# SchusterLab/quantum-optimal-control

Measured on AMD Instinct MI355X. Metric: GRAPE iterations/sec (fwd+bwd+Adam) at n=32 k=4 steps=500, higher is better.
Workload: dtype f64; 1 GPU; C2 3-transmon-size unitary gate: n=32 k=4 steps=500 m=8 Taylor(T,s)=(5,3), 64 independent control seeds per GPU (aggregate over seeds), reg_coeffs={}; seeds_per_gpu=64, total_seeds=64, chunks=16, stream_groups=1, ranks_seen=1, fidelities_gathered=64, devices_distinct=1, transport=single process, transport_fallback=False

## Files before the change

### quantum-optimal-control_amd/csrc/qoc_engine.hip

```cpp
#include "../../include/qoc.h"

#include <hip/hip_runtime.h>

#include <cmath>
#include <cstdarg>
#include <cstdio>
#include <cstdlib>
#include <cstring>
#include <memory>
#include <string>
#include <type_traits>
#include <vector>

#include "qoc_common.h"
#include "qoc_kernels_finish.h"
#include "qoc_kernels_generic.h"
#include "qoc_kernels_mfma.h"
#include "qoc_kernels_st.h"
#include "qoc_kernels_gemm.h"
#include "qoc_gemm_ts.h"
#include "qoc_small.h"
#include "qoc_ensemble.h"
#include "qoc_transfer.h"
#include "qoc_control_map.h"
// ... 1741 lines not shown
}

int qoc_get_member_weights(qoc_handle e, double* pi) {
    CHECK_H(e);
    if (!e->ens_E) return fail(QOC_ERR_STATE, "qoc_get_member_weights: not an ensemble engine (qoc_create_ensemble, qoc_create_shaped)");
    if (!pi) return fail(QOC_ERR_INVALID, "qoc_get_member_weights: null output");
    const size_t E = (size_t)e->ens_E, cnt = (size_t)e->g.B * E;
    if (!risk_on(e)) {
        for (size_t i = 0; i < cnt; ++i) pi[i] = e->ens_wt[i % E];
        return QOC_OK;
    }
    HIP_TRY(hipStreamSynchronize(e->stream));
    HIP_TRY(hipMemcpy(pi, e->risk_pi, cnt * sizeof(double), hipMemcpyDeviceToHost));
    return QOC_OK;
}

int qoc_get_trajectory_gradient(qoc_handle e, double* dLdu) {
    CHECK_H(e);
    if (!e->ens_E) return fail(QOC_ERR_STATE, "qoc_get_trajectory_gradient: not an ensemble engine (qoc_create_ensemble)");
    if (!dLdu) return fail(QOC_ERR_INVALID, "qoc_get_trajectory_gradient: null output");
    if (!e->evaluated) return fail(QOC_ERR_STATE, "qoc_get_trajectory_gradient: nothing evaluated yet");
    HIP_TRY(hipStreamSynchronize(e->stream));
    HIP_TRY(hipMemcpy(dLdu, e->d.dLdu, (size_t)e->d.B * e->d.k * e->d.steps * sizeof(double), hipMemcpyDeviceToHost));
    return QOC_OK;
}

int qoc_get_member_final_unitary(qoc_handle e, double* Uf) {
    CHECK_H(e);
    if (!e->ens_E) return fail(QOC_ERR_STATE, "qoc_get_member_final_unitary: not an ensemble engine (qoc_create_ensemble)");
    if (e->lb.on) return fail(QOC_ERR_STATE, "qoc_get_member_final_unitary: an open engine has no final unitary (qoc_get_member_final_density)");
    if (!Uf) return fail(QOC_ERR_INVALID, "qoc_get_member_final_unitary: null output");
    if (e->d.state_transfer) return fail(QOC_ERR_STATE, "qoc_get_member_final_unitary: state-transfer mode has no final unitary");
    if (!e->evaluated) return fail(QOC_ERR_STATE, "qoc_get_member_final_unitary: nothing evaluated yet");
    TRY(refresh_final(e));
    HIP_TRY(hipStreamSynchronize(e->stream));
    HIP_TRY(hipMemcpy(Uf, e->d.Xfinal, (size_t)e->d.B * e->d.n * e->d.n * sizeof(cplx), hipMemcpyDeviceToHost));
    return QOC_OK;
}

int qoc_profile_enable(qoc_handle e, int32_t on) {
    CHECK_H(e);
    TRY(prof_collect(e));
    e->profiling = on != 0;
    e->prof_ms = 0.0;
    e->prof_launches = 0;
    return QOC_OK;
}

int qoc_profile_read(qoc_handle e, const char** kernel_name, int64_t* launches, double* total_ms) {
    CHECK_H(e);
    TRY(prof_collect(e));
    if (kernel_name)
        *kernel_name = e->path == QOC_PATH_SPARSE ? "k_sp_forward" : e->path == QOC_PATH_LINDBLAD ? "k_lb_forward" : e->path == QOC_PATH_SMALL ? "k_small_iter (whole iterations)"
                       : e->path == QOC_PATH_GEMM ? (e->gm.route == QOC_GEMM_DIRECT ? "k_gemm_taylor_chain (backward chain + sources + gradient products)"
                           : e->gm.N <= 64 ? "k_gemm_expm_fused (+ product tree)" : "k_zgemm_wg + k_zgemm32 (batched matexp sequence)")
                       : e->path == QOC_PATH_MFMA ? e->mp.expm_name
                       : e->path == QOC_PATH_ST_FUSED ? "k_st_fwd_fused" : (e->d.state_transfer ? "k_st_fwd_generic" : "k_expm_generic");
    if (launches) *launches = e->prof_launches;
    if (total_ms) *total_ms = e->prof_ms;
    return QOC_OK;
}

int qoc_time_iterations(qoc_handle e, const qoc_adam_params* p, int32_t iters, double* elapsed_ms) {
    CHECK_H(e);
    HIP_TRY(hipStreamSynchronize(e->stream));
    HIP_TRY(hipEventRecord(e->t0, e->stream));
    TRY(qoc_iterate(e, p, iters));
    HIP_TRY(hipEventRecord(e->t1, e->stream));
    HIP_TRY(hipEventSynchronize(e->t1));
    float ms = 0.f;
    HIP_TRY(hipEventElapsedTime(&ms, e->t0, e->t1));
    if (elapsed_ms) *elapsed_ms = ms;
    return QOC_OK;
}

int qoc_path_in_use(qoc_handle e) { return e ? e->path : QOC_ERR_INVALID; }
int qoc_chunks_in_use(qoc_handle e) { return e ? e->chunks : QOC_ERR_INVALID; }

int qoc_plan_describe(qoc_handle e, char* buf, int32_t len) {
    if (!e || !buf || len < 1) return fail(QOC_ERR_INVALID, "qoc_plan_describe: null handle or buffer");
    char tmp[768];
    if (e->path == QOC_PATH_MFMA) {
        int w = snprintf(tmp, sizeof tmp, "path=mfma nt=%d expm=%d chunks=%d sweeps=%s", e->mf.NT, e->mp.expm_variant, e->mf.C, e->mp.sweeps);
        if (e->mp.expm_variant == 8) w += snprintf(tmp + w, sizeof tmp - w, " expm_hermitian=%d", e->mp.expm_hermitian);
        snprintf(tmp + w, sizeof tmp - w, " mem_policy=%d", e->mp.mem_policy);
    } else if (e->path == QOC_PATH_GEMM) {
        const QocGemm& g = e->gm;
        const bool direct = g.route == QOC_GEMM_DIRECT;
        int w = snprintf(tmp, sizeof tmp, "path=gemm route=%s chunks=%d slices_per_chunk=%d chains=%s",
                         direct ? "direct" : (e->d.state_transfer ? "propagator" : "unitary"), g.NC, g.S, qoc_gemm_chain_routes(g) ? "persistent" : "launches");
        if (g.ts_G > 0) w += snprintf(tmp + w, sizeof tmp - w, " time_shards=%d time_rank=%d", g.ts_G, g.ts_rank);
        if (direct) snprintf(tmp + w, sizeof tmp - w, " taylor_chain=%s",
                             g.sq_chain ? "squared" : g.dpp_packed ? "packed"
                             : g.dpp_chain ? (g.dpp_cw == 10 ? "columns40" : g.dpp_cw == 12 ? "columns48" : g.dpp_cw == 14 ? "columns56" : "full")
                             : "butterfly");
    } else if (e->path == QOC_PATH_LINDBLAD) {
        snprintf(tmp, sizeof tmp, "path=lindblad collapse=%d pairs=%d lds=%zu", e->lb.c, e->lb.R, e->lb.lds_bytes);
    } else if (e->path == QOC_PATH_SPARSE) {
        const QocSparse& sp = e->sp;
        int w = snprintf(tmp, sizeof tmp, "path=sparse nnz=%lld ell=", sp.stored);
        for (size_t j = 0; j < e->sp_widths.size() && w < 320; ++j) w += snprintf(tmp + w, sizeof tmp - w, j ? ",%d" : "%d", e->sp_widths[j]);
        w += snprintf(tmp + w, sizeof tmp - w, " vector_home=%s lds=%zu threads=%d grad_grid=%d", sp.home == 1 ? "lds" : "global", sp.lds_bytes, sp.threads, sp.grad_grid);
        if (e->sp_fleet_entry) snprintf(tmp + w, sizeof tmp - w, " rows=%s merged_width=%d", sp.merged ? "merged" : "per_operator", sp.Wm);
    } else if (e->path == QOC_PATH_SMALL) {
        snprintf(tmp, sizeof tmp, "path=small n_pad=%d rows=%d slices_per_row=%d workgroups=%d state_sources=%d lds_kb=%d", e->sm.N, e->sm.R, e->sm.L, e->sm.G,
            e->sm.src ? 1 : 0, (int)((e->sm.lds_bytes + 1023) / 1024));
    } else {
        snprintf(tmp, sizeof tmp, "path=%s", e->path == QOC_PATH_ST_FUSED ? "st_fused" : "generic");
    }
    auto add = [&tmp](const char* fmt, auto... a) { const size_t w = strlen(tmp); snprintf(tmp + w, sizeof tmp - w, fmt, a...); };
    const int ks = sets(e).k * sets(e).steps;
    const TailKind tail = tail_kind(e);
    if (tail == TAIL_IN_LAUNCH) add(" tail=%s", "in_launch");
    else if (tail == TAIL_SPLIT) add(" tail=split%d", e->fin_S);
    else if (tail == TAIL_SPLIT_PARTIALS) add(" tail=split%d_partials", e->fin_S);
    else if (tail == TAIL_LATENCY_FUSED) add(" tail=latency_fused_%s", ks <= QF_E * (int)e->mp.grad_lat.block.x ? "regs" : "memory");
    else {
        const int threads = ks >= 2048 ? 1024 : QOC_BLOCK, qfe = tail == TAIL_FINISH8 ? 8 : QF_E;
        add(" tail=finish%d_%s", threads, tail == TAIL_FINISH8 ? "regs8" : (ks <= qfe * threads ? "regs" : "memory"));
    }
    if (e->ens_E) add(" members=%d perturbations=%d", e->ens_E, e->en.q);
    if (e->fleet_F) add(" devices=%d", e->fleet_F);
    if (e->shaped) add(" samples=%d band=%d", e->sh.P, e->sh.band);
    if (e->mapped) add(" terms=%d degree=%d", e->cm.r, e->cm.D);
    add(" gradient=%s", e->xg.on ? "exact" : "first_order");
    if (e->xg.on) add(" exact_variant=%s exact_lds=%zu exact_grid=%d", e->xg.lds ? "lds" : "global", e->xg.lds_bytes, e->xg.grid);
    if (e->lb.on && e->lb.nc > 0) add(" running_costs=%d", e->lb.nc);
    if (e->en.tr) add(" traces=1");
    snprintf(buf, (size_t)len, "%s", tmp);
    return QOC_OK;
}

}

#include "qoc_comm.h"
```

### quantum-optimal-control_amd/csrc/qoc_mfma_backward.hip

```cpp
#include "qoc_kernels_mfma.h"
#include "qoc_plan_limits.h"
#include "qoc_mfma_backward.h"
#include "qoc_mfma_downup.h"

template <int NT>
static const char* qoc_resolve_backward(QocMfmaPlan& p, const QocMfma& mf, const QocDev& d, bool split_grad, int mem_policy) {
    const unsigned items = d.B * mf.C, g4 = (items + 3) / 4, slices = d.B * d.steps;
    const bool src = d.n_forb > 0 || d.has_speed, fast = mf.variant != 1;
    const QocOneOf<2, 4> mq{mf.mq <= 2 ? 2 : 4};
    const QocOneOf<5, 4> kc{d.k == 5 ? 5 : 4};
    const QocOneOf<8, 7, 6, 5> qa{qoc_active_strips(d.n)};
    if (src && mf.C > 1) {
        const unsigned wpg = mf.lat_sources ? 1 : 4;
        if (NT == 2 && fast) qoc_pick([&](auto MQ, auto QA) { p.offsets.set(k_mfma_bwd_offsets2<MQ, false, QA>, (items + wpg - 1) / wpg, 64 * wpg); }, mq, qa);
        else p.offsets.set(k_mfma_bwd_offsets<NT>, g4, 256);
    }
    if constexpr (NT == 2) if (fast && d.k <= 5) {
        if (mf.lat_sources) {
            qoc_pick([&](auto MQ, auto KC) {
                p.sweep_groups.set(k_mfma_backward3<MQ, true, KC, 2>, d.B * mf.NG, 128, mf.bwd_lds3);
                p.sweep.set(k_mfma_backward3<MQ, true, KC, 1>, items, 128, mf.bwd_lds3);
            }, mq, kc);
            return p.sweep_groups.reserve() && p.sweep.reserve() ? nullptr : "MFMA path: cannot reserve LDS for the two-level backward kernel";
        }
// ... 44 lines not shown
        C = NT == 2 ? QOC_PLAN_CHUNK_ITEMS / d.Bplan : (QOC_PLAN_CHUNK_ITEMS + d.Bplan - 1) / d.Bplan;
        if (C > (NT == 2 ? QOC_PLAN_CHUNKS_MAX_NT2 : QOC_PLAN_CHUNKS_MAX)) C = NT == 2 ? QOC_PLAN_CHUNKS_MAX_NT2 : QOC_PLAN_CHUNKS_MAX;
    }
    mf.latency = mf.variant == 5;
    if (mf.latency && chunks_req <= 0) C = (d.steps + 7) / 8;
    if (C > d.steps) C = d.steps;
    if (C > (mf.latency ? 16 * QOC_MAXC : QOC_MAXC)) C = mf.latency ? 16 * QOC_MAXC : QOC_MAXC;
    if (C < 1) C = 1;
    int L = (d.steps + C - 1) / C;
    C = (d.steps + L - 1) / L;
    mf.C = C; mf.L = L;
    mf.G = 0; mf.NG = 0;
    mf.lat_sources = mf.latency && (d.n_forb > 0 || d.has_speed);
    if (mf.latency) {
        int G = 8;
        while (G * G < C) ++G;
        mf.G = G; mf.NG = (C + G - 1) / G;
    }
    mf.mq = (d.m + 3) / 4;
    {
        double f = 1.0;
        for (int j = 0; j < 24; ++j) { if (j > 0) f *= (double)j; mf.invfact[j] = 1.0 / f; }
    }
    std::vector<cplx> hd((size_t)(d.k + 1) * FR), ht((size_t)(d.k + 1) * FR), u0(FR);
    for (int kk = 0; kk <= d.k; ++kk) {
        qoc_to_fragD(Hs_host + (size_t)kk * d.n * d.n, d.n, false, hd.data() + (size_t)kk * FR, NT);
        qoc_to_fragD(Hs_host + (size_t)kk * d.n * d.n, d.n, true, ht.data() + (size_t)kk * FR, NT);
    }
    std::vector<cplx> u0h((size_t)d.n * d.n);
    if (hipMemcpy(u0h.data(), d.U0, u0h.size() * sizeof(cplx), hipMemcpyDeviceToHost) != hipSuccess) { msg = "U0 readback failed"; return -2; }
    qoc_to_fragD(u0h.data(), d.n, false, u0.data(), NT);
    auto up = [&](cplx** dst, const std::vector<cplx>& src) -> bool {
        void* p = nullptr;
        if (hipMalloc(&p, src.size() * sizeof(cplx)) != hipSuccess) return false;
        allocs.push_back(p);
        if (hipMemcpy(p, src.data(), src.size() * sizeof(cplx), hipMemcpyHostToDevice) != hipSuccess) return false;
        *dst = (cplx*)p;
        return true;
    };
    if (!up(&mf.HfD, hd) || !up(&mf.HfT, ht) || !up(&mf.U0fD, u0)) { msg = "MFMA path: constant upload failed"; return -3; }
    {
        const int T = d.T < 1 ? 1 : (d.T > 22 ? 22 : d.T);
        mf.psigma = std::pow(mf.invfact[T], 1.0 / (double)T);
        for (int j = 0; j < 24; ++j) mf.pcoef[j] = mf.invfact[j] * std::pow(mf.psigma, -(double)j);
        mf.pcoef[T] = 1.0;
        const double sc = mf.psigma / (double)(1 << d.s);
        std::vector<cplx> hs(hd);
        for (auto& v : hs) { v.x *= sc; v.y *= sc; }
        if (!up(&mf.HsD, hs)) { msg = "MFMA path: constant upload failed"; return -3; }
    }
    std::vector<std::pair<cplx**, size_t>> wanted;
    auto al = [&](cplx** dst, size_t count) -> bool { wanted.emplace_back(dst, (count * sizeof(cplx) + 4095) & ~(size_t)4095); return true; };
    mf.skew_c = 5 * 16;
    mf.skew_b = 3 * 16;
    const size_t nk = (size_t)d.B * ((size_t)d.steps * FR + (size_t)C * mf.skew_c + mf.skew_b), np = (size_t)d.B * C * FR;
    mf.store_T = !((NT == 2 || NT == 3) && mf.variant != 1) || mf.latency;
    const bool split_grad = (NT > 2 || (NT == 2 && d.k >= 6)) && mf.variant != 1;
    if (split_grad && !al(&mf.LamD, (size_t)d.B * d.steps * 16 * NT * 16)) { msg = "MFMA path: out of device memory"; return -3; }
    { const int kg = NT >= 4 ? 2 : 4; mf.grad_lds = (size_t)(d.k < kg ? d.k : kg) * FR * sizeof(cplx); }
    mf.grad_rt = NT >= 2 && split_grad && d.k <= 8 && !qoc_exp_is("QOC_GRAD_RT", 0);
    if (mf.grad_rt) {
        mf.grad_lds = (size_t)((d.k + 3) & ~3) * NT * 256 * sizeof(cplx);
        if (!al((cplx**)&mf.gpart, ((size_t)NT * d.B * d.k * d.steps + 1) / 2)) { msg = "MFMA path: out of device memory"; return -3; }
    }
    if (mf.updown && !al(&mf.LamL, (size_t)d.B * d.steps * NT * (mf.mq <= 2 ? 2 : 4) * 64)) { msg = "MFMA path: out of device memory"; return -3; }
    if (mf.lat_sources && !al(&mf.Goff, (size_t)d.B * mf.NG * 4 * NT * 64)) { msg = "MFMA path: out of device memory"; return -3; }
    const bool bnd = (NT == 2 || NT == 3) && mf.variant != 1 && !mf.latency;
    const bool bnd_adj = bnd && NT == 2 && d.k <= 5 && !(d.n_forb > 0 || d.has_speed);
    mf.updown = mf.updown && bnd_adj;
    const size_t nbnd = (size_t)d.B * C * NT * (mf.mq <= 2 ? 2 : 4) * 64;
    if ((bnd && !al(&mf.BndF, nbnd)) || (bnd_adj && !al(&mf.BndA, nbnd))) { msg = "MFMA path: out of device memory"; return -3; }
    const bool dressed = d.n_forb > 0 && d.forbid_dressed;
    mf.lat_src_fast = mf.lat_sources && !(dressed && d.n_forb > 4);
    mf.lat_dressed = mf.lat_src_fast && dressed;
    if (mf.lat_src_fast) {
        const size_t vec = (size_t)NT * (mf.mq <= 2 ? 2 : 4) * 64;
        if (!al(&mf.AoffL, (size_t)d.B * C * vec) || !al(&mf.GoffL, (size_t)d.B * mf.NG * vec) || !al(&mf.LamS, (size_t)d.B * d.steps * vec) ||
            !al((cplx**)&mf.loss_part, (size_t)d.B * (d.steps + 1))) { msg = "MFMA path: out of device memory"; return -3; }
    }
    if (mf.latency && (!al(&mf.GfD, (size_t)d.B * mf.NG * FR) || !al(&mf.GfT, (size_t)d.B * mf.NG * FR) || !al(&mf.TfD, (size_t)d.B * FR) ||
                       !al(&mf.PsiL, (size_t)d.B * d.steps * NT * (mf.mq <= 2 ? 2 : 4) * 64) ||
                       !al(&mf.LamL, (size_t)d.B * d.steps * NT * (mf.mq <= 2 ? 2 : 4) * 64))) { msg = "MFMA path: out of device memory"; return -3; }
    if (!al(&mf.KfD, nk) || (mf.store_T && !al(&mf.KfT, nk)) || !al(&mf.PfD, np) || !al(&mf.PfT, np) || !al(&mf.Aoff, (size_t)d.B * C * 4 * NT * 64)) { msg = "MFMA path: out of device memory"; return -3; }
    {
        size_t total = 0;
        for (auto& w : wanted) total += w.second;
        char* arena = nullptr;
        if (hipMalloc((void**)&arena, qoc_arena_bytes(total)) != hipSuccess) { msg = "MFMA path: out of device memory"; return -3; }
        allocs.push_back(arena);
        size_t off = 0;
        for (auto& w : wanted) { *w.first = (cplx*)(arena + off); off += w.second; }
        const size_t xl = (size_t)d.B * d.steps * NT * (mf.mq <= 2 ? 2 : 4) * 64 * sizeof(cplx);
        if (mf.PsiL && (hipMemset(mf.PsiL, 0, xl) != hipSuccess || hipMemset(mf.LamL, 0, xl) != hipSuccess)) { msg = "MFMA path: clearing PsiL / LamL failed"; return -2; }
        if (NT == 2 && d.n <= 28 && (hipMemset(mf.KfD, 0, nk * sizeof(cplx)) != hipSuccess || (mf.KfT && hipMemset(mf.KfT, 0, nk * sizeof(cplx)) != hipSuccess))) {
            msg = "MFMA path: clearing the propagator buffers failed"; return -2;
        }
    }
    const size_t pads = (size_t)4 * 16 * (16 * NT + 1) * sizeof(cplx);
    const size_t hbytes = (size_t)d.k * FR * sizeof(cplx);
    mf.h_in_lds = (hbytes + pads) <= 160 * 1024;
    mf.bwd_lds = pads + (mf.h_in_lds ? hbytes : 0);
    {
        const int kc = d.k == 5 ? 5 : 4;
        mf.bwd_lds3 = (size_t)kc * FR * sizeof(cplx) + (size_t)8 * 2 * 16 * B2_LDP * sizeof(cplx) + 4 * 2 * 2 * 4 * kc * sizeof(double);
    }
    if (mf.latency) {
        void* p = nullptr;
        if (hipMalloc(&p, (size_t)d.B * sizeof(unsigned)) != hipSuccess) { msg = "MFMA path: out of device memory"; return -3; }
        allocs.push_back(p);
        if (hipMemset(p, 0, (size_t)d.B * sizeof(unsigned)) != hipSuccess) { msg = "MFMA path: clearing the arrival counters failed"; return -2; }
        mf.lat_count = (unsigned*)p;
    }
    if (mf.updown) {
        const int kc = d.k == 5 ? 5 : 4, mqv = mf.mq <= 2 ? 2 : 4;
        mf.du_lds = (size_t)kc * FR * sizeof(cplx) + (size_t)8 * 4 * mqv * F2_LDP * sizeof(cplx) + (size_t)4 * 2 * NT * mqv * 64 * sizeof(cplx) +
                    (size_t)8 * 4 * kc * sizeof(double) + 8 * sizeof(int);
    }
    plan = QocMfmaPlan{};
    const bool lat_own = mf.latency && (!mf.lat_sources || mf.lat_src_fast);
    plan.engine_loss = !mf.updown && !lat_own;
    plan.tail_fusable = lat_own;
    plan.own_controls = mf.latency && NT == 2;
    plan.uscale_in_loss = !mf.latency && !mf.updown;
    plan.final_on_readback = mf.latency || mf.updown;
    plan.final_from_groups = mf.latency;
    plan.inter_on_readback = lat_own || mf.updown;
    plan.sweeps = mf.latency ? (mf.lat_sources ? "latency_sources" : "latency")
                  : mf.updown ? "downup" : (split_grad ? (mf.grad_rt ? "row_tile_gradient" : "split") : (mf.variant == 1 || NT == 1 || NT == 4 ? "one_wave" : "pair"));
    plan.expm_hermitian = !qoc_all_antihermitian(Hs_host, d.n, d.k + 1) || qoc_exp_is("QOC_EXPM_HERM", 0) ? 0 : (qoc_exp_is("QOC_EXPM_HERM", 2) ? 2 : 1);
    const int mem_policy = qoc_exp_is("QOC_MEM_POLICY", 0) ? 0 : 1;
    plan.mem_policy = mem_policy;
    const char* err = qoc_mfma_resolve_expm(plan, mf, d);
    qoc_mfma_resolve_expm_inplace(plan, mf, d);
    qoc_mfma_resolve_forward(plan, mf, d);
    if (!err) err = qoc_mfma_resolve_latency(plan, mf, d);
    if (!err && !lat_own) qoc_pick([&](auto NTc) { err = qoc_resolve_backward<NTc>(plan, mf, d, split_grad, mem_policy); }, QocOneOf<1, 2, 3, 4>{NT});
    if (err) { msg = err; return -2; }
    return 0;
}

void qoc_mfma_launch_backward(const QocMfmaPlan& p, const QocMfma& mf, const QocDev& d, hipStream_t s) {
    if (p.tail_fusable) { qoc_mfma_latency_gradient(p, mf, d, nullptr, s); return; }
    p.offsets.run(s, d, mf);
    p.costates.run(s, d, mf);
    p.sweep_groups.run(s, d, mf);
    p.sweep.run(s, d, mf);
    p.sweep1.run(s, d, mf, 0);
    p.grad.run(s, d, mf);
    p.grad_sum.run(s, d, mf, mf.NT);
}
```

### quantum-optimal-control_amd/csrc/qoc_mfma_expm_inplace.h

```cpp
#pragma once
#include <type_traits>
#include <utility>
#include "qoc_mfma_frag.h"

#define ILDS (16 * NT + 5)
#define SLDS 21

#ifndef QOC_INPLACE_PIPE
#define QOC_INPLACE_PIPE 0
#endif
#ifndef QOC_INPLACE_STAGE2
#define QOC_INPLACE_STAGE2 0
#endif
#ifndef QOC_INPLACE_SWAP
#define QOC_INPLACE_SWAP 0
#endif
#ifndef QOC_EXPM_KSTORE
#define QOC_EXPM_KSTORE PLAIN
#endif
constexpr bool qoc_expm_has_policy = QOC_MEM(QOC_EXPM_KSTORE) != QocMem::PLAIN;
#ifndef QOC_LAP
#define QOC_LAP(ph)
#define QOC_LAP_INIT
#define QOC_LAP_DONE
// ... 50 lines not shown
            const int st = ib * QS + kb;
            fetch(st + RA);
            fence();
            if (PLANES && ib > 0) {
#pragma unroll
                for (int q = kb - off; q >= 0 && q < 3 * NT; q += QS) {
                    const int J = q / 3, w = q % 3;
                    if (w < 2) ((double*)(wbase + 16 * J * ILDS + 4 * pib))[w] = ring.ppl[w][J];
                    else wbases[16 * J * ILDS + 4 * pib] = ring.ppl[2][J];
                    fence();
                }
            } else if (kb >= off && kb < off + 2 * NT) {
                const int q = kb - off;
                if ((q & 1) == 0) wbase[16 * (q >> 1) * ILDS + 4 * pib] = ring.pri[q >> 1];
                else wbases[16 * (q >> 1) * ILDS + 4 * pib] = ring.psu[q >> 1];
                fence();
            }
            if constexpr (half) {
                if (kb == 1) { fence(); mir = side[(4 * (ib - 2 * NT) + (lane >> 4)) * SLDS + (lane & 15)]; fence(); }
            }
            const cplx v = ring.v[st & 3];
            const double vs = ring.s[st & 3];
#pragma unroll
            for (int J = J0; J < NT; ++J) {
                const bool ab = !(SYM == 1 && half && J == 0);
                if (kb == 0) {
                    if (ab) a[J] = __builtin_amdgcn_mfma_f64_4x4x4f64(v.x, P.re[J][kb], preset ? a[J] : 0.0, 0, 0, 0);
                    if (ab) b[J] = __builtin_amdgcn_mfma_f64_4x4x4f64(v.y, P.im[J][kb], 0.0, 0, 0, 0);
                    c[J] = __builtin_amdgcn_mfma_f64_4x4x4f64(vs, P.su[J][kb], preset ? c[J] : 0.0, 0, 0, 0);
                } else {
                    if (ab) a[J] = __builtin_amdgcn_mfma_f64_4x4x4f64(v.x, P.re[J][kb], a[J], 0, 0, 0);
                    if (ab) b[J] = __builtin_amdgcn_mfma_f64_4x4x4f64(v.y, P.im[J][kb], b[J], 0, 0, 0);
                    c[J] = __builtin_amdgcn_mfma_f64_4x4x4f64(vs, P.su[J][kb], c[J], 0, 0, 0);
                }
            }
            if constexpr (QOC_INPLACE_PIPE && ib > 0) {
                if (kb == 0) {
                    __builtin_amdgcn_sched_barrier(0);
                    static_assert(!PLANES || !QOC_INPLACE_PIPE, "plane epilogues with the deferred combine are not wired up");
                    if constexpr (!PLANES) epi(std::integral_constant<int, ib - 1>{}, acc[(ib - 1) & 1][0], acc[(ib - 1) & 1][1], acc[(ib - 1) & 1][2], ring.pri, ring.psu);
                    __builtin_amdgcn_sched_barrier(0);
                }
            }
            if constexpr (RELOAD_IN) {
                if (ib == 0 && kb == (QS > 2 * NT + 1 ? 2 * NT : 2 * NT - 1)) {
                    fence();
#pragma unroll
                    for (int J = 0; J < NT; ++J) load_strip<NT, true>(img, imgs, lane, P, J, QS - 1);
                    fence();
                }
            }
            if constexpr (RELOAD_OUT) {
                if (ib == QS - 1 && kb < QS - 1) {
                    fence();
#pragma unroll
                    for (int J = 0; J < NT; ++J) load_strip<NT, true>(img, imgs, lane, P, J, kb);
                    fence();
                }
            }
        }
        if constexpr (!QOC_INPLACE_PIPE || ib == QS - 1) {
            __builtin_amdgcn_sched_barrier(0);
            if constexpr (SYM == 1) {
                if constexpr (half) { a[0] = mir.x; b[0] = mir.y; }
                else { fence(); side[(lane & 15) * SLDS + 4 * ib + (lane >> 4)] = cmake(a[1], b[1]); fence(); }
            }
            if constexpr (PLANES) {
                epi(ibc, a, b, c, ring.ppl[0], ring.ppl[1], ring.ppl[2]);
                if constexpr (ib == QS - 1) {
#pragma unroll
                    for (int J = 0; J < NT; ++J) { ring.pri[J] = cmake(ring.ppl[0][J], ring.ppl[1][J]); ring.psu[J] = ring.ppl[2][J]; }
                }
            } else if constexpr (SYM == 2) epi(ibc, a, b, c, ring.pri, ring.psu, mir);
            else epi(ibc, a, b, c, ring.pri, ring.psu);
            __builtin_amdgcn_sched_barrier(0);
        }
    }, std::make_integer_sequence<int, QS>{});
#pragma unroll
    for (int st = NS; st < NSP; ++st) { fetch(st + RA); fence(); }
}

__device__ __forceinline__ const cplx* frag_at(const cplx* F, int f) { return F + (f & ~3) * 64; }
__device__ __forceinline__ cplx* frag_at(cplx* F, int f) { return F + (f & ~3) * 64; }

template <QocMem POL, int NT, int ib>
__device__ __forceinline__ void store_kstrip(cplx* Kout, int J, unsigned ulane, const cplx v) {
    constexpr int QS = 4 * NT;
    if constexpr (POL == QocMem::PLAIN) frag_at(Kout, J * QS + ib)[((J * QS + ib) & 3) * 64 + ulane] = v;
    else for_each([&](auto Jc) {
        constexpr int f = decltype(Jc)::value * QS + ib;
        if (J == decltype(Jc)::value) qoc_st16_at<POL, (f & 3) * 64>(frag_at(Kout, f), ulane, v);
    }, std::make_integer_sequence<int, NT>{});
}

}

template <int KC, bool EVEN, bool S0, int QA = 8, int HERM = 0, int POL = 0>
__global__ void __launch_bounds__(64, 1) k_mfma_expm_inplace(QocDev d, QocMfma mf) {
    using namespace qoc_inplace;
    constexpr int NT = 2, QS = 4 * NT;
    constexpr QocMem KST = POL ? QOC_MEM(QOC_EXPM_KSTORE) : QocMem::PLAIN;
    static_assert(!HERM || (QA == 8 && !QOC_INPLACE_SWAP && (HERM == 1 || !EVEN)), "symmetric products: the full 32 x 32 problem; even/odd chain: Taylor order 5");
    __shared__ __attribute__((aligned(16))) cplx img[QNP * ILDS];
    __shared__ __attribute__((aligned(16))) double imgs[QNP * ILDS];
    __shared__ __attribute__((aligned(16))) cplx side[HERM ? 16 * SLDS : 1];
    const int lane = threadIdx.x;
    const unsigned ulane = threadIdx.x;
    const int b = blockIdx.x / mf.C, c = blockIdx.x - b * mf.C;
    if (d.skip_done && d.done[b]) return;
    QOC_LAP_INIT
    const int t0 = c * mf.L, t1 = min(t0 + mf.L, d.steps);
    const int dlt = (lane & 15) - (lane >> 4);
    double idv[4];
#pragma unroll
    for (int r = 0; r < 4; ++r) idv[r] = dlt == 4 * r ? 1.0 : 0.0;
    const int mm = d.T >> 1;
    constexpr bool even = EVEN;
    const int nH = even ? mm - 1 : mm;
    const double p_c0 = even ? mf.pcoef[2 * mm - 2] : mf.pcoef[2 * mm], p_c1 = even ? mf.pcoef[2 * mm - 1] : 1.0;

    Set<NT> SA, SB, R;
    constexpr bool SWAP = QOC_INPLACE_SWAP && KC <= 4;
    Ring<NT> ring;
    auto diag = [&](int J, int ib) -> double { return (ib >> 2) == J ? idv[ib & 3] : 0.0; };
    auto no_init = [](auto, double (&)[NT], double (&)[NT]) { return std::false_type{}; };

#pragma unroll
    for (int J = 0; J < NT; ++J)
#pragma unroll
        for (int ib = 0; ib < QS; ++ib) {
            R.re[J][ib] = diag(J, ib); R.im[J][ib] = 0.0; R.su[J][ib] = diag(J, ib);
            if (SWAP && ib >= QA) { SB.re[J][ib] = diag(J, ib); SB.im[J][ib] = 0.0; SB.su[J][ib] = diag(J, ib); }
        }

    const cplx* hk[KC + 1];
    hk[0] = mf.HsD;
#pragma unroll
    for (int kk = 0; kk < KC; ++kk) hk[kk + 1] = mf.HsD + (size_t)(kk < d.k ? kk + 1 : 0) * QFR;
    auto coeffs = [&](int t, double (&ck)[KC]) {
#pragma unroll
        for (int kk = 0; kk < KC; ++kk) ck[kk] = kk < d.k ? d.u[((size_t)b * d.k + kk) * d.steps + t] : 0.0;
    };
    auto assemble = [&](const cplx (&h)[KC + 1], const double (&ck)[KC], double& re, double& im) {
        re = h[0].x; im = h[0].y;
#pragma unroll
        for (int kk = 0; kk < KC; ++kk) { re = fma(ck[kk], h[kk + 1].x, re); im = fma(ck[kk], h[kk + 1].y, im); }
    };
    auto combine = [](double a, double bq, double cq, double& re, double& im, double& su) { re = a - bq; su = fma(-2.0, bq, cq); im = su - re; };

    {
        double ck[KC];
        coeffs(t0, ck);
#pragma unroll
        for (int J = 0; J < NT; ++J)
#pragma unroll
            for (int ib = 0; ib < QA; ++ib) {
                cplx h[KC + 1];
#pragma unroll
                for (int kk = 0; kk <= KC; ++kk) h[kk] = frag_at(hk[kk], J * QS + ib)[((J * QS + ib) & 3) * 64 + ulane];
                double re, im;
                assemble(h, ck, re, im);
                SA.re[J][ib] = re; SA.im[J][ib] = im; SA.su[J][ib] = re + im;
                if (ib == QA - 1) { ring.pri[J] = cmake(re, im); ring.psu[J] = re + im; }
                else {
                    const int o = (16 * J + (lane & 15)) * ILDS + 4 * ib + (lane >> 4);
                    img[o] = cmake(re, im); imgs[o] = re + im;
                }
                fence();
            }
        {
            const cplx* base = img + (lane >> 4) * ILDS + (lane & 3);
            const double* bases = imgs + (lane >> 4) * ILDS + (lane & 3);
#pragma unroll
            for (int st = 0; st < 3; ++st) { ring.v[st] = base[4 * st * ILDS]; ring.s[st] = bases[4 * st * ILDS]; }
        }
        fence();
    }
    QOC_LAP(0)

    auto slice = [&](Set<NT>& SB, Set<NT>& R, int t) __attribute__((always_inline)) {
        cplx* Kout = mf.KfD + kitem(mf, d.steps, b, t);
        Set<NT>& SQ = *(HERM == 2 ? &SA : &SB);
        if constexpr (HERM == 2) {
        const double o0 = mf.pcoef[1], o1 = mf.pcoef[3], e2 = mf.pcoef[4], e0 = mf.pcoef[0], g1 = mf.pcoef[2] - e2 * o1;
        auto side_store = [&](int ib, double re, double im) { fence(); side[(lane & 15) * SLDS + 4 * ib + (lane >> 4)] = cmake(re, im); fence(); };
        product<NT, QA, false, false, false, 2>(img, imgs, lane, ring, SA, no_init,
                                        [&](auto ibc, double (&a)[NT], double (&bq)[NT], double (&cq)[NT], cplx (&ori)[NT], double (&osu)[NT], const cplx& mir) {
            constexpr int ib = decltype(ibc)::value;
#pragma unroll
            for (int J = 0; J < NT; ++J) {
                double re, im, su;
                if (ib >= 2 * NT && J == 0) { re = mir.x; im = mir.y; su = re + im; }
                else combine(a[J], bq[J], cq[J], re, im, su);
                SB.re[J][ib] = re; SB.im[J][ib] = im; SB.su[J][ib] = su;
                ori[J] = cmake(re, im); osu[J] = su;
                if (ib < 2 * NT && J == 1) side_store(ib, re, -im);
            }
        }, side);
        QOC_LAP(1)
        product<NT, QA, false, false, false, 2>(img, imgs, lane, ring, SB,
                                        [&](auto ibc, double (&a)[NT], double (&cq)[NT]) {
            constexpr int ib = decltype(ibc)::value;
#pragma unroll
            for (int J = ib >= 2 * NT ? 1 : 0; J < NT; ++J) {
                a[J] = o1 * SB.re[J][ib];
                cq[J] = o1 * SB.su[J][ib];
            }
            return std::true_type{};
        },
                                        [&](auto ibc, double (&a)[NT], double (&bq)[NT], double (&cq)[NT], cplx (&ori)[NT], double (&osu)[NT], const cplx& mir) {
            constexpr int ib = decltype(ibc)::value;
#pragma unroll
            for (int J = 0; J < NT; ++J) {
// ... 8 lines not shown
        auto load_o = [&](int ib, double (&r)[NT], double (&su)[NT]) {
            fence();
#pragma unroll
            for (int J = ib >= 2 * NT ? 1 : 0; J < NT; ++J) {
                const int o = (16 * J + (lane & 15)) * ILDS + 4 * ib + (lane >> 4);
                r[J] = ((const double*)(img + o))[0]; su[J] = imgs[o];
            }
            fence();
        };
        load_o(0, Or[0], Os[0]);
        product<NT, QA, false, !S0, false, 2>(img, imgs, lane, ring, SA,
                                        [&](auto ibc, double (&a)[NT], double (&cq)[NT]) {
            constexpr int ib = decltype(ibc)::value;
#pragma unroll
            for (int J = ib >= 2 * NT ? 1 : 0; J < NT; ++J) {
                double er = fma(e2, Or[ib & 1][J], g1 * SB.re[J][ib]), es = fma(e2, Os[ib & 1][J], g1 * SB.su[J][ib]);
                if ((ib >> 2) == J) { er = fma(e0, diag(J, ib), er); es = fma(e0, diag(J, ib), es); }
                a[J] = fma(o0, SA.re[J][ib], er); cq[J] = fma(o0, SA.su[J][ib], es);
                if (ib < 2 * NT && J == 1) { Er = er; Es = es; }
            }
            if constexpr (ib + 1 < QA) load_o(ib + 1, Or[(ib + 1) & 1], Os[(ib + 1) & 1]);
            return std::true_type{};
        },
                                        [&](auto ibc, double (&a)[NT], double (&bq)[NT], double (&cq)[NT], cplx (&ori)[NT], double (&osu)[NT], const cplx& mir) {
            constexpr int ib = decltype(ibc)::value;
#pragma unroll
            for (int J = 0; J < NT; ++J) {
                double re, im, su;
                if (ib >= 2 * NT && J == 0) { re = mir.x; im = mir.y; su = re + im; }
                else combine(a[J], bq[J], cq[J], re, im, su);
                ori[J] = cmake(re, im); osu[J] = su;
                if constexpr (S0) store_kstrip<KST, NT, ib>(Kout, J, ulane, ori[J]);
                if (ib < 2 * NT && J == 1) side_store(ib, fma(2.0, Er, -re), fma(-2.0, Es - Er, im));
            }
        }, side);
        QOC_LAP(2)
        } else {
        product<NT, QA, false, false, true, HERM == 1 ? 1 : 0>(img, imgs, lane, ring, SA, no_init,
                                        [&](auto ibc, double (&a)[NT], double (&bq)[NT], double (&cq)[NT], double (&ore)[NT], double (&oim)[NT], double (&osu)[NT]) {
            constexpr int ib = decltype(ibc)::value;
#pragma unroll
            for (int J = 0; J < NT; ++J) {
                double re, im, su;
                combine(a[J], bq[J], cq[J], re, im, su);
                SB.re[J][ib] = re; SB.im[J][ib] = im; SB.su[J][ib] = su;
                if constexpr (even) {
                    ore[J] = re + fma(p_c1, SA.re[J][ib], p_c0 * diag(J, ib));
                    oim[J] = fma(p_c1, SA.im[J][ib], im);
                    osu[J] = ore[J] + oim[J];
                } else if ((ib >> 2) == J) {
                    ore[J] = fma(p_c0, diag(J, ib), SA.re[J][ib]); oim[J] = SA.im[J][ib]; osu[J] = fma(p_c0, diag(J, ib), SA.su[J][ib]);
                } else {
                    ore[J] = SA.re[J][ib]; oim[J] = SA.im[J][ib]; osu[J] = SA.su[J][ib];
                }
            }
        }, HERM == 1 ? side : nullptr);
        QOC_LAP(1)
        for (int i = nH - 1; i >= 0; --i) {
            const double d0 = mf.pcoef[2 * i], d1 = mf.pcoef[2 * i + 1];
            auto init = [&](auto ibc, double (&a)[NT], double (&cq)[NT]) {
                constexpr int ib = decltype(ibc)::value;
#pragma unroll
                for (int J = 0; J < NT; ++J) {
                    a[J] = fma(d1, SA.re[J][ib], d0 * diag(J, ib));
                    cq[J] = fma(d1, SA.su[J][ib], d0 * diag(J, ib));
                }
                return std::true_type{};
            };
            auto epi = [&](auto ibc, double (&a)[NT], double (&bq)[NT], double (&cq)[NT], cplx (&ori)[NT], double (&osu)[NT]) {
                constexpr int ib = decltype(ibc)::value;
#pragma unroll
                for (int J = 0; J < NT; ++J) {
                    double re, im, su;
                    combine(a[J], bq[J], cq[J], re, im, su);
                    ori[J] = cmake(re, im); osu[J] = su;
                    if constexpr (S0) { if (i == 0) store_kstrip<KST, NT, ib>(Kout, J, ulane, ori[J]); }
                }
            };
            if (i > 0) product<NT, QA, false, false, false>(img, imgs, lane, ring, SB, init, epi);
            else product<NT, QA, false, true, false>(img, imgs, lane, ring, SB, init, epi);
        }
        QOC_LAP(2)
        }
        for (int sq = 0; sq < d.s; ++sq) {
            const bool kout = sq == d.s - 1;
            product<NT, QA, true, true, false>(img, imgs, lane, ring, SQ, no_init,
                                    [&](auto ibc, double (&a)[NT], double (&bq)[NT], double (&cq)[NT], cplx (&ori)[NT], double (&osu)[NT]) {
                constexpr int ib = decltype(ibc)::value;
#pragma unroll
                for (int J = 0; J < NT; ++J) {
                    double re, im, su;
                    combine(a[J], bq[J], cq[J], re, im, su);
                    ori[J] = cmake(re, im); osu[J] = su;
                    if (kout) store_kstrip<KST, NT, ib>(Kout, J, ulane, ori[J]);
                }
            });
        }
        QOC_LAP(3)
        {
            double ck[KC];
            coeffs(min(t + 1, d.steps - 1), ck);
            constexpr int HD = QOC_INPLACE_STAGE2 ? 2 : 1;
            cplx h[HD][NT][KC + 1];
            auto stage = [&](int ib) {
#pragma unroll
                for (int J = 0; J < NT; ++J)
#pragma unroll
                    for (int kk = 0; kk <= KC; ++kk) h[ib % HD][J][kk] = frag_at(hk[kk], J * QS + ib)[((J * QS + ib) & 3) * 64 + ulane];
            };
            stage(0);
            if constexpr (HD == 2) stage(1);
            Set<NT>& RN = SB;
            product<NT, QA, false, false, false>(img, imgs, lane, ring, R, no_init,
                                      [&](auto ibc, double (&a)[NT], double (&bq)[NT], double (&cq)[NT], cplx (&ori)[NT], double (&osu)[NT]) {
                constexpr int ib = decltype(ibc)::value;
#pragma unroll
                for (int J = 0; J < NT; ++J) {
                    double re, im;
                    assemble(h[ib % HD][J], ck, re, im);
                    ori[J] = cmake(re, im); osu[J] = re + im;
                }
                if constexpr (ib + HD < QA) stage(ib + HD);
#pragma unroll
                for (int J = 0; J < NT; ++J) combine(a[J], bq[J], cq[J], RN.re[J][ib], RN.im[J][ib], RN.su[J][ib]);
            });
            QOC_LAP(4)
            if constexpr (!SWAP) {
#pragma unroll
                for (int J = 0; J < NT; ++J)
#pragma unroll
                    for (int ib = 0; ib < QA; ++ib) { R.re[J][ib] = SB.re[J][ib]; R.im[J][ib] = SB.im[J][ib]; R.su[J][ib] = SB.su[J][ib]; }
            }
            fence();
#pragma unroll
            for (int J = 0; J < NT; ++J) {
#pragma unroll
                for (int ib = 0; ib < QA - 1; ++ib) load_strip<NT, false>(img, imgs, lane, SA, J, ib);
                SA.re[J][QA - 1] = ring.pri[J].x; SA.im[J][QA - 1] = ring.pri[J].y; SA.su[J][QA - 1] = ring.psu[J];
            }
            fence();
            QOC_LAP(5)
        }
    };
    if constexpr (SWAP) {
    Set<NT>* Rfin = &R;
    for (int t = t0; t < t1; t += 2) {
        slice(SB, R, t); Rfin = &SB;
        if (t + 1 < t1) { slice(R, SB, t + 1); Rfin = &R; }
    }
    if (Rfin != &R) {
#pragma unroll
        for (int J = 0; J < NT; ++J)
#pragma unroll
            for (int ib = 0; ib < QS; ++ib) { R.re[J][ib] = SB.re[J][ib]; R.im[J][ib] = SB.im[J][ib]; }
    }
    } else {
        for (int t = t0; t < t1; ++t) slice(SB, R, t);
    }
    const size_t pitem = (size_t)b * mf.C + c;
#pragma unroll
    for (int J = 0; J < NT; ++J)
#pragma unroll
        for (int ib = 0; ib < QS; ++ib) frag_at(mf.PfD + pitem * QFR, J * QS + ib)[((J * QS + ib) & 3) * 64 + ulane] = cmake(R.re[J][ib], R.im[J][ib]);
    wave_lds_fence();
#pragma unroll
    for (int J = 0; J < NT; ++J)
#pragma unroll
        for (int ib = 0; ib < QS; ++ib) img[(16 * J + (lane & 15)) * ILDS + 4 * ib + (lane >> 4)] = cmake(R.re[J][ib], R.im[J][ib]);
    wave_lds_fence();
#pragma unroll
    for (int J = 0; J < NT; ++J)
#pragma unroll
        for (int q = 0; q < QS; ++q) frag_at(mf.PfT + pitem * QFR, J * QS + q)[((J * QS + q) & 3) * 64 + ulane] = img[(4 * q + (lane >> 4)) * ILDS + 16 * J + (lane & 15)];
    QOC_LAP(6)
    QOC_LAP_DONE
}
```

### quantum-optimal-control_amd/csrc/qoc_mfma_expm_inplace.hip

```cpp
#include "qoc_kernels_mfma.h"
#include "qoc_mfma_expm_inplace.h"

void qoc_mfma_resolve_expm_inplace(QocMfmaPlan& p, const QocMfma& mf, const QocDev& d) {
    const int herm = (p.expm_variant == 8 && d.T == 5 && qoc_active_strips(d.n) == 8) ? p.expm_hermitian : 0;
    p.expm_hermitian = herm;
    const int pol = (p.expm_variant == 8 && qoc_expm_has_policy && d.k <= 4) ? p.mem_policy : 0;
    p.mem_policy = pol;
    if (p.expm_variant != 8) return;
    qoc_pick([&](auto KC, auto EVEN, auto S0, auto QA, auto HERM, auto POL) {
        if constexpr (HERM != 0 && (EVEN != 0 || QA != 8)) return;
        else if constexpr (POL != 0 && (!qoc_expm_has_policy || KC != 4)) return;
        else p.expm.set(k_mfma_expm_inplace<KC, EVEN != 0, S0 != 0, QA, HERM, POL>, d.B * mf.C, 64);
    }, QocOneOf<4, 8>{d.k <= 4 ? 4 : 8}, QocOneOf<1, 0>{(d.T & 1) == 0}, QocOneOf<1, 0>{d.s == 0}, QocOneOf<8, 7, 6, 5>{qoc_active_strips(d.n)}, QocOneOf<1, 2, 0>{herm},
       QocOneOf<1, 0>{pol});
}
```

### quantum-optimal-control_amd/csrc/qoc_mfma_frag.h

```cpp
#pragma once
#include <string>
#include <vector>
#include "qoc_common.h"

#define QOC_NP 32
#define QOC_MAXC 64
#define QNP (16 * NT)
#define QQS (4 * NT)
#define QLDR (16 * NT + 1)
#define QFR (256 * NT * NT)
#define F2_LDP 33
static inline int qoc_active_strips(int n) { return n > 28 ? 8 : (n > 24 ? 7 : (n > 20 ? 6 : 5)); }
static inline int qoc_active_strips_lat(int n) { return n > 16 ? qoc_active_strips(n) : (n > 8 ? 4 : 2); }

typedef double d4 __attribute__((ext_vector_type(4)));
#define QMFMA(a, b, c) __builtin_amdgcn_mfma_f64_16x16x4f64((a), (b), (c), 0, 0, 0)

struct CTile { d4 re, im; };
template <int NT> struct AFragT { double re[NT][4 * NT], im[NT][4 * NT]; };

struct QocMfma {
    int C = 1;
    int L = 1;
    int mq = 4;
    int NT = 2;
    int FR = 1024;
    double invfact[24];
    double pcoef[24];
    double psigma = 1.0;
    cplx* HsD = nullptr;
    cplx* HfD = nullptr;
    cplx* HfT = nullptr;
    cplx* U0fD = nullptr;
    cplx* KfD = nullptr;
    cplx* KfT = nullptr;
    bool store_T = true;
    cplx* PfD = nullptr;
    cplx* PfT = nullptr;
    cplx* BndF = nullptr;
    cplx* BndA = nullptr;
    bool updown = false;
    size_t du_lds = 0;
    cplx* Aoff = nullptr;
    cplx* Goff = nullptr;
    cplx* LamD = nullptr;
    size_t grad_lds = 0;
    double* gpart = nullptr;
    int grad_rt = 0;
    size_t bwd_lds = 0, bwd_lds3 = 0;
    bool h_in_lds = true;
    int variant = 0;
    int G = 0, NG = 0;
    cplx* GfD = nullptr;
    cplx* TfD = nullptr;
    cplx* PsiL = nullptr;
    cplx* LamL = nullptr;
    cplx* LamS = nullptr;
    cplx* AoffL = nullptr;
    cplx* GoffL = nullptr;
    bool lat_dressed = false;
    bool exp_rows_qa_full = false, exp_lat_qa8 = false, exp_lat_offsets_own = false;
    bool lat_src_fast = false;
    double* loss_part = nullptr;
    unsigned* lat_count = nullptr;
    cplx* GfT = nullptr;
    bool latency = false;
    bool lat_sources = false;
    int skew_c = 0, skew_b = 0;
};

__device__ __forceinline__ size_t kitem(const QocMfma& mf, int steps, int b, int t) {
    return (size_t)b * ((size_t)steps * mf.FR + (size_t)mf.C * mf.skew_c + mf.skew_b) + (size_t)t * mf.FR + (size_t)(t / mf.L) * mf.skew_c;
}

enum class QocMem { PLAIN, NT, WT };
#define QOC_MEM_(x) QocMem::x
#define QOC_MEM(x) QOC_MEM_(x)
typedef double qoc_d2 __attribute__((ext_vector_type(2)));
template <QocMem POL>
__device__ __forceinline__ cplx qoc_ld16(const cplx* p) {
    static_assert(POL != QocMem::WT, "write-through is a store policy");
    if constexpr (POL == QocMem::NT) { const qoc_d2 v = __builtin_nontemporal_load((const qoc_d2*)p); return cmake(v.x, v.y); }
    else return *p;
}
template <QocMem POL>
__device__ __forceinline__ void qoc_st16(cplx* p, const cplx v) {
    if constexpr (POL == QocMem::NT) __builtin_nontemporal_store((qoc_d2){v.x, v.y}, (qoc_d2*)p);
    else if constexpr (POL == QocMem::WT) {
        asm volatile("global_store_dwordx4 %0, %1, off sc0 sc1\n\ts_nop 1" :: "v"(p), "v"((qoc_d2){v.x, v.y}) : "memory");
    } else *p = v;
}
template <QocMem POL, int IMM>
__device__ __forceinline__ void qoc_st16_at(cplx* base, unsigned lane, const cplx v) {
    static_assert(IMM >= 0 && IMM < 256, "13-bit signed immediate of the global instructions");
    if constexpr (POL == QocMem::WT) {
        asm volatile("s_nop 4\n\tglobal_store_dwordx4 %0, %1, %2 offset:%3 sc0 sc1\n\ts_nop 1" :: "v"(lane * 16u), "v"((qoc_d2){v.x, v.y}), "s"(base), "n"(IMM * 16) : "memory");
    } else qoc_st16<POL>(base + (IMM + lane), v);
}


template <int NT, bool CONJ, int QA = 4 * NT>
__device__ __forceinline__ void afrag_load(const cplx* __restrict__ F, int lane, AFragT<NT>& A) {
#pragma unroll
    for (int I = 0; I < NT; ++I)
#pragma unroll
        for (int q = 0; q < QA; ++q) {
            const cplx v = F[(I * QQS + q) * 64 + lane];
            A.re[I][q] = v.x; A.im[I][q] = CONJ ? -v.y : v.y;
        }
}
template <int NT>
__device__ __forceinline__ void colblock_load(const cplx* __restrict__ F, int J, int lane, CTile p[NT]) {
#pragma unroll
    for (int Ib = 0; Ib < NT; ++Ib)
#pragma unroll
        for (int r = 0; r < 4; ++r) {
            const cplx v = F[(J * QQS + 4 * Ib + r) * 64 + lane];
            p[Ib].re[r] = v.x; p[Ib].im[r] = v.y;
        }
}
template <int NT>
__device__ __forceinline__ void colblock_store(cplx* __restrict__ F, int J, int lane, const CTile p[NT]) {
#pragma unroll
    for (int Ib = 0; Ib < NT; ++Ib)
#pragma unroll
        for (int r = 0; r < 4; ++r) F[(J * QQS + 4 * Ib + r) * 64 + lane] = cmake(p[Ib].re[r], p[Ib].im[r]);
}
template <int NT>
__device__ __forceinline__ void afrag_store_half(cplx* __restrict__ F, int J, int lane, const AFragT<NT>& A) {
#pragma unroll
    for (int q = 0; q < QQS; ++q) {
        double re = A.re[0][q], im = A.im[0][q];
#pragma unroll
        for (int Jc = 1; Jc < NT; ++Jc)
            if (Jc == J) { re = A.re[Jc][q]; im = A.im[Jc][q]; }
        F[(J * QQS + q) * 64 + lane] = cmake(re, im);
    }
}
template <int NT>
__device__ __forceinline__ void colblock_identity(int J, int lane, CTile p[NT]) {
    const int dlt = (lane & 15) - (lane >> 4);
#pragma unroll
    for (int Ib = 0; Ib < NT; ++Ib)
#pragma unroll
        for (int r = 0; r < 4; ++r) {
            p[Ib].re[r] = (Ib == J && dlt == 4 * r) ? 1.0 : 0.0; p[Ib].im[r] = 0.0;
        }
}

template <int NT, int QA = 4 * NT>
__device__ __forceinline__ void mm_colblock(const AFragT<NT>& A, const CTile p[NT], CTile out[NT]) {
// ... 125 lines not shown
```

### quantum-optimal-control_amd/csrc/qoc_mfma_plan.h

```cpp
#pragma once
#include "qoc_pick.h"
#include "qoc_mfma_frag.h"

template <class... A> struct QocLaunch {
    void (*fn)(A...) = nullptr;
    dim3 grid, block;
    size_t lds = 0;
    void set(void (*f)(A...), unsigned g, unsigned b, size_t l = 0) { fn = f; grid = dim3(g); block = dim3(b); lds = l; }
    void run(hipStream_t s, const A&... a) const { if (fn) hipLaunchKernelGGL(fn, grid, block, lds, s, a...); }
    bool reserve() const { return !fn || !lds || hipFuncSetAttribute((const void*)fn, hipFuncAttributeMaxDynamicSharedMemorySize, (int)lds) == hipSuccess; }
};

struct QocMfmaPlan {
    using K1 = QocLaunch<QocDev>;
    using K2 = QocLaunch<QocDev, QocMfma>;
    using K3 = QocLaunch<QocDev, QocMfma, int>;
    using KScan = QocLaunch<QocDev, QocMfma, int, int, const cplx*, const cplx*, int>;
    using KChain = QocLaunch<QocDev, QocMfma, const cplx*, int, int, int, cplx*, int, const cplx*, cplx*>;
    using KGradLat = QocLaunch<QocDev, QocMfma, QocAdamDev, int>;
    K2 expm;
    KChain chain_chunks, chain_groups;
    KScan scan;
    K2 forward;
    K1 uscale;
    K3 sweep_lat;
    K2 loss_lat;
    K3 sweep_unpack;
    K2 offsets, costates, sweep_groups, sweep;
    K3 sweep1;
    K2 grad;
    K3 grad_sum;
    K3 src_chunks, src_groups, src_total;
    KGradLat grad_lat;
    KChain final_chain;
    K2 final_unpack;
    KScan final_scan;
    K1 final_uscale;
    K3 inter_unpack;
    K2 inter_forward;
    int MQ = 4, scan_flags = 0, final_scan_flags = 0, sweep_offsets = 0;
    bool engine_loss = true;
    bool tail_fusable = false;
    bool own_controls = false;
    bool uscale_in_loss = false;
    bool final_on_readback = false;
    bool final_from_groups = false;
    bool inter_on_readback = false;
    const char* sweeps = "";
    int expm_variant = 1;
    int expm_hermitian = 0;
    int mem_policy = 0;
    const char* expm_name = "";
};
```

Before: 62680 GRAPE iterations/s.

## Park running chunk product in global memory during expm squarings

Adds a PARK variant of the in-place MFMA expm kernel. The running chunk propagator product R (re, im and the sum term) is stored in global memory (PfD plus a new Rsu buffer) and reloaded into the SA register set, so SA can be reused during the squarings and fewer register sets stay live at once. The aim is to cut register pressure and spills in the one-wave-per-block kernel. In exchange it adds global loads and stores with fences on every slice, plus an extra device allocation. It is on by default unless QOC_EXPM_PARK=0.

```diff
diff --git a/quantum-optimal-control_amd/csrc/qoc_engine.hip b/quantum-optimal-control_amd/csrc/qoc_engine.hip
--- a/quantum-optimal-control_amd/csrc/qoc_engine.hip
+++ b/quantum-optimal-control_amd/csrc/qoc_engine.hip
@@ -1847,7 +1847,7 @@
     char tmp[768];
     if (e->path == QOC_PATH_MFMA) {
         int w = snprintf(tmp, sizeof tmp, "path=mfma nt=%d expm=%d chunks=%d sweeps=%s", e->mf.NT, e->mp.expm_variant, e->mf.C, e->mp.sweeps);
-        if (e->mp.expm_variant == 8) w += snprintf(tmp + w, sizeof tmp - w, " expm_hermitian=%d", e->mp.expm_hermitian);
+        if (e->mp.expm_variant == 8) w += snprintf(tmp + w, sizeof tmp - w, " expm_hermitian=%d expm_park=%d", e->mp.expm_hermitian, e->mp.expm_park);
         snprintf(tmp + w, sizeof tmp - w, " mem_policy=%d", e->mp.mem_policy);
     } else if (e->path == QOC_PATH_GEMM) {
         const QocGemm& g = e->gm;
diff --git a/quantum-optimal-control_amd/csrc/qoc_mfma_backward.hip b/quantum-optimal-control_amd/csrc/qoc_mfma_backward.hip
--- a/quantum-optimal-control_amd/csrc/qoc_mfma_backward.hip
+++ b/quantum-optimal-control_amd/csrc/qoc_mfma_backward.hip
@@ -150,6 +150,8 @@
                        !al(&mf.PsiL, (size_t)d.B * d.steps * NT * (mf.mq <= 2 ? 2 : 4) * 64) ||
                        !al(&mf.LamL, (size_t)d.B * d.steps * NT * (mf.mq <= 2 ? 2 : 4) * 64))) { msg = "MFMA path: out of device memory"; return -3; }
     if (!al(&mf.KfD, nk) || (mf.store_T && !al(&mf.KfT, nk)) || !al(&mf.PfD, np) || !al(&mf.PfT, np) || !al(&mf.Aoff, (size_t)d.B * C * 4 * NT * 64)) { msg = "MFMA path: out of device memory"; return -3; }
+    const bool park = NT == 2 && qoc_mfma_expm_variant(mf, d) == 8 && d.s > 0 && !qoc_exp_is("QOC_EXPM_PARK", 0);
+    if (park && !al((cplx**)&mf.Rsu, np / 2)) { msg = "MFMA path: out of device memory"; return -3; }
     {
         size_t total = 0;
         for (auto& w : wanted) total += w.second;
@@ -198,6 +200,7 @@
     plan.expm_hermitian = !qoc_all_antihermitian(Hs_host, d.n, d.k + 1) || qoc_exp_is("QOC_EXPM_HERM", 0) ? 0 : (qoc_exp_is("QOC_EXPM_HERM", 2) ? 2 : 1);
     const int mem_policy = qoc_exp_is("QOC_MEM_POLICY", 0) ? 0 : 1;
     plan.mem_policy = mem_policy;
+    plan.expm_park = mf.Rsu ? 1 : 0;
     const char* err = qoc_mfma_resolve_expm(plan, mf, d);
     qoc_mfma_resolve_expm_inplace(plan, mf, d);
     qoc_mfma_resolve_forward(plan, mf, d);
diff --git a/quantum-optimal-control_amd/csrc/qoc_mfma_expm_inplace.h b/quantum-optimal-control_amd/csrc/qoc_mfma_expm_inplace.h
--- a/quantum-optimal-control_amd/csrc/qoc_mfma_expm_inplace.h
+++ b/quantum-optimal-control_amd/csrc/qoc_mfma_expm_inplace.h
@@ -156,6 +156,20 @@
 
 __device__ __forceinline__ const cplx* frag_at(const cplx* F, int f) { return F + (f & ~3) * 64; }
 __device__ __forceinline__ cplx* frag_at(cplx* F, int f) { return F + (f & ~3) * 64; }
+struct LaneOff {
+    unsigned c[4], d[2];
+    __device__ __forceinline__ void set(unsigned lane) {
+#pragma unroll
+        for (int g = 0; g < 4; ++g) c[g] = lane * 16u + 4096u * g;
+#pragma unroll
+        for (int g = 0; g < 2; ++g) d[g] = lane * 8u + 4096u * g;
+        asm volatile("" : "+v"(c[0]), "+v"(c[1]), "+v"(c[2]), "+v"(c[3]), "+v"(d[0]), "+v"(d[1]));
+    }
+};
+__device__ __forceinline__ const cplx& lane_at(const cplx* F, int f, const LaneOff& o) { return *(const cplx*)((const char*)F + (size_t)o.c[f >> 2] + (f & 3) * 1024); }
+__device__ __forceinline__ cplx& lane_at(cplx* F, int f, const LaneOff& o) { return *(cplx*)((char*)F + (size_t)o.c[f >> 2] + (f & 3) * 1024); }
+__device__ __forceinline__ const double& lane_at(const double* F, int f, const LaneOff& o) { return *(const double*)((const char*)F + (size_t)o.d[f >> 3] + (f & 7) * 512); }
+__device__ __forceinline__ double& lane_at(double* F, int f, const LaneOff& o) { return *(double*)((char*)F + (size_t)o.d[f >> 3] + (f & 7) * 512); }
 
 template <QocMem POL, int NT, int ib>
 __device__ __forceinline__ void store_kstrip(cplx* Kout, int J, unsigned ulane, const cplx v) {
@@ -169,11 +183,12 @@
 
 }
 
-template <int KC, bool EVEN, bool S0, int QA = 8, int HERM = 0, int POL = 0>
+template <int KC, bool EVEN, bool S0, int QA = 8, int HERM = 0, int POL = 0, int PARK = 0>
 __global__ void __launch_bounds__(64, 1) k_mfma_expm_inplace(QocDev d, QocMfma mf) {
     using namespace qoc_inplace;
     constexpr int NT = 2, QS = 4 * NT;
     constexpr QocMem KST = POL ? QOC_MEM(QOC_EXPM_KSTORE) : QocMem::PLAIN;
+    static_assert(!PARK || (!S0 && HERM != 2 && !QOC_INPLACE_SWAP), "parked chunk product: SA must be free during the squarings; one slice body");
     static_assert(!HERM || (QA == 8 && !QOC_INPLACE_SWAP && (HERM == 1 || !EVEN)), "symmetric products: the full 32 x 32 problem; even/odd chain: Taylor order 5");
     __shared__ __attribute__((aligned(16))) cplx img[QNP * ILDS];
     __shared__ __attribute__((aligned(16))) double imgs[QNP * ILDS];
@@ -199,10 +214,21 @@
     auto diag = [&](int J, int ib) -> double { return (ib >> 2) == J ? idv[ib & 3] : 0.0; };
     auto no_init = [](auto, double (&)[NT], double (&)[NT]) { return std::false_type{}; };
 
+    cplx* Rp = PARK ? mf.PfD + ((size_t)b * mf.C + c) * QFR : nullptr;
+    double* Rs = PARK ? mf.Rsu + ((size_t)b * mf.C + c) * QFR : nullptr;
+    LaneOff lo;
+    if constexpr (PARK) lo.set(ulane);
 #pragma unroll
     for (int J = 0; J < NT; ++J)
 #pragma unroll
         for (int ib = 0; ib < QS; ++ib) {
+            if constexpr (PARK) {
+                if (ib < QA) {
+                    lane_at(Rp, J * QS + ib, lo) = cmake(diag(J, ib), 0.0);
+                    lane_at(Rs, J * QS + ib, lo) = diag(J, ib);
+                }
+                continue;
+            }
             R.re[J][ib] = diag(J, ib); R.im[J][ib] = 0.0; R.su[J][ib] = diag(J, ib);
             if (SWAP && ib >= QA) { SB.re[J][ib] = diag(J, ib); SB.im[J][ib] = 0.0; SB.su[J][ib] = diag(J, ib); }
         }
@@ -377,6 +403,19 @@
         }
         QOC_LAP(2)
         }
+        if constexpr (PARK) {
+            fence();
+            lo.set(ulane);
+#pragma unroll
+            for (int J = 0; J < NT; ++J)
+#pragma unroll
+                for (int ib = 0; ib < QA; ++ib) {
+                    const cplx v = lane_at((const cplx*)Rp, J * QS + ib, lo);
+                    SA.re[J][ib] = v.x; SA.im[J][ib] = v.y;
+                    SA.su[J][ib] = lane_at((const double*)Rs, J * QS + ib, lo);
+                }
+            fence();
+        }
         for (int sq = 0; sq < d.s; ++sq) {
             const bool kout = sq == d.s - 1;
             product<NT, QA, true, true, false>(img, imgs, lane, ring, SQ, no_init,
@@ -401,8 +440,12 @@
 #pragma unroll
                 for (int J = 0; J < NT; ++J)
 #pragma unroll
-                    for (int kk = 0; kk <= KC; ++kk) h[ib % HD][J][kk] = frag_at(hk[kk], J * QS + ib)[((J * QS + ib) & 3) * 64 + ulane];
+                    for (int kk = 0; kk <= KC; ++kk) {
+                        if constexpr (PARK) h[ib % HD][J][kk] = lane_at(hk[kk], J * QS + ib, lo);
+                        else h[ib % HD][J][kk] = frag_at(hk[kk], J * QS + ib)[((J * QS + ib) & 3) * 64 + ulane];
+                    }
             };
+            if constexpr (PARK) lo.set(ulane);
             stage(0);
             if constexpr (HD == 2) stage(1);
             Set<NT>& RN = SB;
@@ -416,11 +459,21 @@
                     ori[J] = cmake(re, im); osu[J] = re + im;
                 }
                 if constexpr (ib + HD < QA) stage(ib + HD);
-#pragma unroll
-                for (int J = 0; J < NT; ++J) combine(a[J], bq[J], cq[J], RN.re[J][ib], RN.im[J][ib], RN.su[J][ib]);
+                if constexpr (PARK) {
+#pragma unroll
+                    for (int J = 0; J < NT; ++J) {
+                        double re, im, su;
+                        combine(a[J], bq[J], cq[J], re, im, su);
+                        lane_at(Rp, J * QS + ib, lo) = cmake(re, im);
+                        lane_at(Rs, J * QS + ib, lo) = su;
+                    }
+                } else {
+#pragma unroll
+                    for (int J = 0; J < NT; ++J) combine(a[J], bq[J], cq[J], RN.re[J][ib], RN.im[J][ib], RN.su[J][ib]);
+                }
             });
             QOC_LAP(4)
-            if constexpr (!SWAP) {
+            if constexpr (!SWAP && !PARK) {
 #pragma unroll
                 for (int J = 0; J < NT; ++J)
 #pragma unroll
@@ -449,14 +502,28 @@
 #pragma unroll
             for (int ib = 0; ib < QS; ++ib) { R.re[J][ib] = SB.re[J][ib]; R.im[J][ib] = SB.im[J][ib]; }
     }
+    } else if constexpr (PARK) {
+        for (int t = t0; t < t1; ++t) slice(SB, SA, t);
     } else {
         for (int t = t0; t < t1; ++t) slice(SB, R, t);
     }
     const size_t pitem = (size_t)b * mf.C + c;
+    if constexpr (PARK) {
+        fence();
+        lo.set(ulane);
+#pragma unroll
+        for (int J = 0; J < NT; ++J)
+#pragma unroll
+            for (int ib = 0; ib < QS; ++ib) {
+                if (ib < QA) { const cplx v = lane_at((const cplx*)Rp, J * QS + ib, lo); R.re[J][ib] = v.x; R.im[J][ib] = v.y; }
+                else { R.re[J][ib] = diag(J, ib); R.im[J][ib] = 0.0; }
+            }
+        fence();
+    }
 #pragma unroll
     for (int J = 0; J < NT; ++J)
 #pragma unroll
-        for (int ib = 0; ib < QS; ++ib) frag_at(mf.PfD + pitem * QFR, J * QS + ib)[((J * QS + ib) & 3) * 64 + ulane] = cmake(R.re[J][ib], R.im[J][ib]);
+        for (int ib = PARK ? QA : 0; ib < QS; ++ib) frag_at(mf.PfD + pitem * QFR, J * QS + ib)[((J * QS + ib) & 3) * 64 + ulane] = cmake(R.re[J][ib], R.im[J][ib]);
     wave_lds_fence();
 #pragma unroll
     for (int J = 0; J < NT; ++J)
diff --git a/quantum-optimal-control_amd/csrc/qoc_mfma_expm_inplace.hip b/quantum-optimal-control_amd/csrc/qoc_mfma_expm_inplace.hip
--- a/quantum-optimal-control_amd/csrc/qoc_mfma_expm_inplace.hip
+++ b/quantum-optimal-control_amd/csrc/qoc_mfma_expm_inplace.hip
@@ -6,11 +6,14 @@
     p.expm_hermitian = herm;
     const int pol = (p.expm_variant == 8 && qoc_expm_has_policy && d.k <= 4) ? p.mem_policy : 0;
     p.mem_policy = pol;
+    const int park = (p.expm_variant == 8 && d.s > 0 && herm != 2 && mf.Rsu) ? p.expm_park : 0;
+    p.expm_park = park;
     if (p.expm_variant != 8) return;
-    qoc_pick([&](auto KC, auto EVEN, auto S0, auto QA, auto HERM, auto POL) {
+    qoc_pick([&](auto KC, auto EVEN, auto S0, auto QA, auto HERM, auto POL, auto PARK) {
         if constexpr (HERM != 0 && (EVEN != 0 || QA != 8)) return;
         else if constexpr (POL != 0 && (!qoc_expm_has_policy || KC != 4)) return;
-        else p.expm.set(k_mfma_expm_inplace<KC, EVEN != 0, S0 != 0, QA, HERM, POL>, d.B * mf.C, 64);
+        else if constexpr (PARK != 0 && (S0 != 0 || HERM == 2)) return;
+        else p.expm.set(k_mfma_expm_inplace<KC, EVEN != 0, S0 != 0, QA, HERM, POL, PARK>, d.B * mf.C, 64);
     }, QocOneOf<4, 8>{d.k <= 4 ? 4 : 8}, QocOneOf<1, 0>{(d.T & 1) == 0}, QocOneOf<1, 0>{d.s == 0}, QocOneOf<8, 7, 6, 5>{qoc_active_strips(d.n)}, QocOneOf<1, 2, 0>{herm},
-       QocOneOf<1, 0>{pol});
+       QocOneOf<1, 0>{pol}, QocOneOf<1, 0>{park});
 }
diff --git a/quantum-optimal-control_amd/csrc/qoc_mfma_frag.h b/quantum-optimal-control_amd/csrc/qoc_mfma_frag.h
--- a/quantum-optimal-control_amd/csrc/qoc_mfma_frag.h
+++ b/quantum-optimal-control_amd/csrc/qoc_mfma_frag.h
@@ -67,6 +67,7 @@
     bool latency = false;
     bool lat_sources = false;
     int skew_c = 0, skew_b = 0;
+    double* Rsu = nullptr;
 };
 
 __device__ __forceinline__ size_t kitem(const QocMfma& mf, int steps, int b, int t) {
diff --git a/quantum-optimal-control_amd/csrc/qoc_mfma_plan.h b/quantum-optimal-control_amd/csrc/qoc_mfma_plan.h
--- a/quantum-optimal-control_amd/csrc/qoc_mfma_plan.h
+++ b/quantum-optimal-control_amd/csrc/qoc_mfma_plan.h
@@ -50,5 +50,6 @@
     int expm_variant = 1;
     int expm_hermitian = 0;
     int mem_policy = 0;
+    int expm_park = 0;
     const char* expm_name = "";
 };
```

Result: slower. 59980 GRAPE iterations/s (-4.3%).
